# BerserkerMother/Video-Summarization

Measured on AMD Instinct MI355X. Metric: frames/sec scored (whole node), synthetic [B,T=1024,D=1024], higher is better.
Workload: dtype f32; 1 GPU; configs[2]: B=64 videos x T=1024 frames x D=1024 per GPU, scorer cfg M-A (heads 4, d_model 256, layers 4), logits + hidden state; global_batch=64, parallelism=videos sharded over 1 GPU(s), no all_gather of scores

## Files before the change

video-summarization_amd/csrc/vs_forward_plan.h:

```cpp
#pragma once
#include <stddef.h>

#include <cstdio>
#include <string>

#include "vs_scorer.h"

struct VskOptions {
    int skinny_rows;
    int lp_min_rows;
    int train_lp_min_rows;
    int lp_min_rows_fused;
    int attn_w64;
    int lp_store32;
    int lp_mlp_unfused;
    int lp_tail_unfused;
    int lp_qkv_unfused;
    int lp_tile256;
    int lp_embed_unfused;
    int exact_unfused;
    int mlp_abl;
    int attn_w64_checked;
    int attn_w64_abl;
};

enum { VSK_STORE16 = 16, VSK_A16 = 32, VSK_F16 = 64 };

enum { VSW_FRAGMENTS = 1, VSW_F16X3 = 2, VSW_BF16 = 4, VSW_ROWS16 = 8 };

inline bool vsk_mlp_bf16_supported(int d) { return d == 256; }
inline bool vsk_gemm16_supported(int M, int N, int K) { return M > 0 && N > 0 && N % 32 == 0 && K >= 32 && K % 32 == 0; }
inline bool vsk_layer_fused_supported(int M, int d, int skinny_rows) { return d == 256 && M > skinny_rows && M <= (1 << 20); }

enum VsArith { VS_ARITH_EXACT = 0, VS_ARITH_BF16 = 1, VS_ARITH_F16X3 = 2 };
enum VsEmbedForm {
    VS_EMBED_CLS,
    VS_EMBED_BF16_QKV,
    VS_EMBED_SPLITK,
    VS_EMBED_GEMM,
};
enum VsAttentionKernel {
    VS_ATT_PACKED,
    VS_ATT_DH256,
    VS_ATT_SPLITKV,
    VS_ATT_LOWPREC,
    VS_ATT_EXACT,
};
enum VsLayerForm {
    VS_LAYER_RING,
    VS_LAYER_BF16_TAIL,
    VS_LAYER_BF16_MLP,
    VS_LAYER_EXACT_PAIR,
    VS_LAYER_STAGES,
};
enum VsLnForm {
    VS_LN_NONE,
    VS_LN_SPLITK_ROWS,
    VS_LN_GEMM_ROWS,
    VS_LN_FUSED,
};

struct VsForwardIn {
    int d_model, num_heads, num_layers, in_features, max_len;
    int norm_width;
    bool has_pe, has_b_embed;
    int B, T;
    unsigned flags;
    bool cls, packed;
};

struct VsForwardPlan {
    int T, M;
    VsArith linear, attention_arith;
    unsigned families;
    VsEmbedForm embed;
    VsAttentionKernel attention;
    VsLayerForm layer;
    VsLnForm ln1, ln2;
    bool qkv16, ffn16;
    bool next_qkv;
    size_t kv_stride;
    int mode_linear;
    int mode_qkv;
    int mode_ffn;
    int mode_attention;

    bool tail_writes_qkv() const { return next_qkv || layer == VS_LAYER_EXACT_PAIR; }
};

inline int vs_attention_prec(unsigned flags) { return (flags & VS_FLAG_F16X3_ATTENTION) ? 2 : (flags & VS_FLAG_BF16_ATTENTION) ? 1 : 0; }

inline int vs_forward_plan(const VsForwardIn &in, const VskOptions &opt, VsForwardPlan *plan, std::string *err) {
    char msg[192];
    auto fail = [&](int code) { *err = msg; return code; };
    const int d = in.d_model, H = in.num_heads, dh = d / H;
    const unsigned flags = in.flags;
    if (!in.packed && in.has_pe && in.T > in.max_len) {
        snprintf(msg, sizeof msg, "T=%d exceeds the positional table (max_len=%d)", in.T, in.max_len);
        return fail(VS_ERR_INVALID);
    }
    if (in.cls && in.packed) { snprintf(msg, sizeof msg, "packed batches have no class-token form"); return fail(VS_ERR_INVALID); }
    const int T = in.T + (in.cls ? 1 : 0);
    if ((long long)in.B * T > (1ll << 30)) { snprintf(msg, sizeof msg, "B*T too large"); return fail(VS_ERR_INVALID); }
    if ((flags & VS_FLAG_BF16_LINEAR) && (flags & VS_FLAG_F16X3_LINEAR)) {
        snprintf(msg, sizeof msg, "VS_FLAG_BF16_LINEAR and VS_FLAG_F16X3_LINEAR are exclusive");
        return fail(VS_ERR_INVALID);
    }
    if ((flags & (VS_FLAG_BF16_ATTENTION | VS_FLAG_F16X3_ATTENTION)) && dh != 32 && dh != 64 && !((flags & VS_FLAG_BF16_ATTENTION) && dh == 128)) {
        snprintf(msg, sizeof msg, "VS_FLAG_BF16_ATTENTION needs head_dim 32, 64 or 128, VS_FLAG_F16X3_ATTENTION 32 or 64 (got %d)", dh);
        return fail(VS_ERR_INVALID);
    }
    if ((flags & VS_FLAG_BF16_ATTENTION) && (flags & VS_FLAG_F16X3_ATTENTION)) {
        snprintf(msg, sizeof msg, "VS_FLAG_BF16_ATTENTION and VS_FLAG_F16X3_ATTENTION are exclusive");
        return fail(VS_ERR_INVALID);
    }

    VsForwardPlan p{};
    p.T = T;
    p.M = in.B * T;
    const int M = p.M;
    const bool embedded = in.norm_width != d;
    const int aprec = vs_attention_prec(flags);
    p.attention_arith = (VsArith)aprec;
    const bool fused_ok = !embedded && vsk_mlp_bf16_supported(d) && aprec == 1 && !opt.lp_store32 && !opt.lp_mlp_unfused;
    const int lp_min_rows = fused_ok && opt.lp_min_rows_fused < opt.lp_min_rows ? opt.lp_min_rows_fused
                                                                               : opt.lp_min_rows;
    p.linear = (flags & VS_FLAG_F16X3_LINEAR) ? VS_ARITH_F16X3 : ((flags & VS_FLAG_BF16_LINEAR) && M > lp_min_rows) ? VS_ARITH_BF16 : VS_ARITH_EXACT;
    const bool bf16 = p.linear == VS_ARITH_BF16;
    const bool splitk = (flags & VS_FLAG_SPLITK) && !bf16 && !in.packed && !in.cls && M <= opt.skinny_rows && (d == 128 || d == 256 || d == 512);
    const int rows_min = in.cls ? in.B * in.T : M;
    p.families = 0;
    if (bf16) p.families = VSW_BF16;
    else if (rows_min <= opt.skinny_rows) p.families = p.linear == VS_ARITH_F16X3 ? VSW_F16X3 : VSW_FRAGMENTS;
    if (bf16 && d > 256) p.families |= VSW_ROWS16;
    p.ffn16 = bf16 && d <= 256 && !embedded && !opt.lp_store32;
    p.qkv16 = p.ffn16 && aprec == 1;
    const bool mlp16 = bf16 && !embedded && vsk_mlp_bf16_supported(d) && !opt.lp_mlp_unfused && !opt.lp_store32;
    const bool ring = bf16 && aprec == 1 && !in.packed && d > 256 && !opt.lp_store32 && vsk_gemm16_supported(M, d, d);
    p.kv_stride = (p.qkv16 || ring) ? (size_t)M * d / 2 : (size_t)M * d;
    p.next_qkv = mlp16 && p.qkv16 && !opt.lp_qkv_unfused;
    const bool exact_fused = p.linear == VS_ARITH_EXACT && aprec == 0 && !embedded && !splitk && !opt.exact_unfused &&
                             vsk_layer_fused_supported(M, d, opt.skinny_rows) && d % H == 0 && dh % 32 == 0;

    p.embed = in.cls ? VS_EMBED_CLS
            : bf16 && in.has_b_embed && p.next_qkv && in.num_layers > 0 && !opt.lp_embed_unfused ? VS_EMBED_BF16_QKV
            : splitk && in.in_features % 1024 == 0 ? VS_EMBED_SPLITK
            : VS_EMBED_GEMM;
    p.attention = in.packed ? VS_ATT_PACKED
                : dh == 256 ? VS_ATT_DH256
                : splitk && aprec != 1 && (dh == 32 || dh == 64 || dh == 128) ? VS_ATT_SPLITKV
                : aprec ? VS_ATT_LOWPREC
                : VS_ATT_EXACT;
    const VsLnForm ln = (d > 256 || embedded) ? VS_LN_GEMM_ROWS : VS_LN_FUSED;
    p.ln1 = p.ln2 = VS_LN_NONE;
    if (ring) p.layer = VS_LAYER_RING;
    else if (mlp16 && p.qkv16 && !opt.lp_tail_unfused) p.layer = VS_LAYER_BF16_TAIL;
    else if (exact_fused) p.layer = VS_LAYER_EXACT_PAIR;
    else {
        p.layer = mlp16 ? VS_LAYER_BF16_MLP : VS_LAYER_STAGES;
        p.ln1 = splitk && d >= 256 ? VS_LN_SPLITK_ROWS : ln;
        if (!mlp16) p.ln2 = splitk ? VS_LN_SPLITK_ROWS : ln;
    }
    p.mode_linear = p.linear;
    p.mode_qkv = p.qkv16 ? (1 | VSK_STORE16) : p.linear;
    p.mode_ffn = p.ffn16 ? (1 | VSK_STORE16) : p.linear;
    p.mode_attention = (p.qkv16 || ring) ? (1 | VSK_STORE16) : aprec;
    *plan = p;
    return VS_OK;
}

inline int vs_packed_waves(int dh, int aprec, long long r8, long long r4) {
    if (dh == 128) return aprec == 1 ? 8 : 4;
    return (!(aprec != 0 && dh == 32) && r8 * 100 <= r4 * 105) ? 8 : 4;
}
```

video-summarization_amd/csrc/vs_kernels.h:

```cpp
#pragma once
#include <hip/hip_runtime.h>
#include <stdint.h>

#include "vs_forward_plan.h"

int vsk_linear(const float *A, const float *W, const float *Wf, const float *bias, float *C, int M, int N, int K,
               int relu, const float *pe, int T, int bf16, hipStream_t st);
int vsk_linear_gate(const float *A, const float *W, const float *Wf, const float *bias, const float *gate, float scale,
                    float *C, int M, int N, int K, hipStream_t st, int bf16 = 0);
int vsk_linear_relu_dropout(const float *A, const float *W, const float *Wf, const float *bias, float *C, int M, int N,
                            int K, unsigned long long seed, unsigned site, float p, hipStream_t st, int bf16 = 0);
int vsk_pack_fragments(const float *W, float *Wf, int N, int K, hipStream_t st);
int vsk_pack_fragments_f16x3(const float *W, float *Wh, int N, int K, hipStream_t st);
int vsk_qkv(const float *h, const float *Wqkv, const float *Wf, const float *bqkv, float *qkv, int B, int T, int d,
            int H, int bf16, hipStream_t st, float qscale = 1.0f);
int vsk_attention(const float *q, const float *k, const float *v, const uint8_t *mask, float *out,
                  int B, int H, int T, int dh, float scale, hipStream_t st);
int vsk_attention_packed(const float *q, const float *k, const float *v, float *out, int H, int Mtot, int dh,
                         float scale, const int *cu, const int *work, int nwork, int nw, int prec, hipStream_t st);
float vsk_attention_qscale(float scale);
int vsk_attention_bf16(const float *q, const float *k, const float *v, const uint8_t *mask, float *out,
                       int B, int H, int T, int dh, float scale, int prec, hipStream_t st);
int vsk_attention_bf16_w64(const void *q, const void *k, const void *v, const uint8_t *mask, void *out, int B, int H, int T,
                           hipStream_t st);
int vsk_attention_bf16_w64_packed(const void *q, const void *k, const void *v, void *out, int H, int Mtot, const int *cu,
                                  const int *work, int nwork, hipStream_t st);
size_t vsk_attention_probs_workspace_bytes(int B, int H, int T);
int vsk_attention_probs(const float *q, const float *k, const uint8_t *mask, float *maps, float *received, float *entropy,
                        int B, int H, int T, int dh, float scale, void *workspace, hipStream_t st);
int vsk_linear_res_ln(const float *A, const float *W, const float *Wf, const float *bias, const float *res,
                      const float *gamma, const float *beta, float *out, int M, int N, int K,
                      const float *score_w, const float *score_b, int num_classes, int sigmoid,
                      float *scores, int bf16, hipStream_t st);
int vsk_outproj_ln_fc1(const float *att, const float *Wo, const float *bo, const float *res, const float *gamma, const float *beta,
                       float *h1, const float *W1, const float *b1, float *hidden, int M, int d, hipStream_t st);
int vsk_fc2_ln_qkv(const float *hidden, const float *W2, const float *b2, const float *res, const float *gamma, const float *beta,
                   float *out, const float *Wqkv, const float *bqkv, float *qkv, int B, int T, int d, int H, hipStream_t st);
int vsk_rows_res_ln(const float *a, const float *res, const float *gamma, const float *beta, float *out, int M, int d,
                    const float *score_w, const float *score_b, int num_classes, int sigmoid, float *scores,
                    hipStream_t st, void *out16 = nullptr, int dn = 0,
                    int nsplit = 0, const float *pbias = nullptr);
struct VskMatJobs {
    enum { MAX = 24 };
    const float *in[MAX];
    float *out[MAX];
    int rows[MAX], cols[MAX];
    int n;
};
int vsk_pack_fragments_batch(const VskMatJobs &jobs, hipStream_t st);
int vsk_attention_splitkv(const float *q, const float *k, const float *v, const uint8_t *mask, float *out,
                          int B, int H, int T, int dh, float scale, hipStream_t st);
int vsk_linear_parts(const float *A, const float *Wf, float *parts, int M, int N, int K, int nsplit, hipStream_t st,
                     int f16x3 = 0);
int vsk_sum_parts_pe(const float *parts, int nsplit, const float *bias, const float *pe, int T, float *out, int M, int N, hipStream_t st);
int vsk_diag_attention(const float *q, const float *k, const float *v, float *out, int B, int H, int T, float scale,
                       unsigned long long *diag, hipStream_t st);
int vsk_diag_attention_lp(const float *q, const float *k, const float *v, float *out, int B, int H, int T, float scale,
                          int prec, unsigned long long *diag, hipStream_t st);
int vsk_diag_gemm(const float *A, const float *W, const float *bias, float *C, int M, int N, int K,
                  int grid, unsigned long long *diag, hipStream_t st);
size_t vsk_mlp_bf16_image_bytes(int d);
int vsk_pack_mlp_bf16(const float *Wo, const float *W1, const float *W2, void *img, int d, hipStream_t st);
struct VskNextQkv {
    const void *img;
    const float *bqkv;
    void *qkv16;
    int T, H;
    float qscale;
};
size_t vsk_embed_bf16_image_bytes(int d, int K);
int vsk_pack_embed_bf16(const float *W, void *img, int d, int K, hipStream_t st);
int vsk_embed_bf16(const float *x, const void *img, const float *bias, const float *pe, int T, float *out, int M, int d, int K,
                   const VskNextQkv *next, hipStream_t st);
size_t vsk_qkv_bf16_image_bytes(int d);
int vsk_pack_qkv_bf16(const float *Wqkv, void *img, int d, hipStream_t st);
int vsk_mlp_bf16(const float *h, const void *att16, const float *bo, const float *gamma1, const float *beta1,
                 const void *img, const float *b1, const float *b2,
                 const float *gamma, const float *beta, float *out, int M, int d,
                 const float *score_w, const float *score_b, int num_classes, int sigmoid, float *scores,
                 const VskNextQkv *next, hipStream_t st);
int vsk_plan_packed(const int *lengths_dev, int B, int qb, int *cu, int *work, int work_cap, hipStream_t st);
int vsk_gather_rows(const float *pe, const int *cu, int B, int tmax, int d, float *rows, hipStream_t st);
enum { VSK_COPY_MAX_SEGS = 20 };
struct VskCopySegs {
    const float *src[VSK_COPY_MAX_SEGS];
    float *dst[VSK_COPY_MAX_SEGS];
    unsigned n[VSK_COPY_MAX_SEGS];
    int count;
};
int vsk_copy_segments(const VskCopySegs &segs, hipStream_t st);
// ... 11 lines not shown
```

video-summarization_amd/csrc/vs_kernels.hip:

```cpp
#include "vs_train_device.h"
#include "vs_kernels.h"
#include "vs_launch.h"

namespace {

enum { EPI_BIAS = 0, EPI_RELU = 1, EPI_PE = 2, EPI_QKV = 3,
       EPI_GATE = 4,
       EPI_RELU_DROP = 5 };
struct EpiArgs {
    unsigned long long seed;
    unsigned site;
    float p;
    float scale;
};

__device__ __forceinline__ unsigned long long stamp() { return vs_stamp(); }

template <int EPI, int NWM = 2, int DIAG = 0, int NJ = 2, int PREC = 0, int C16 = 0, int KW = 32, int A16 = 0>
__global__ __launch_bounds__(128 * NWM, 2) void gemm_nt_128(
    const float *__restrict__ A, const float *__restrict__ W, const float *__restrict__ bias,
    float *__restrict__ C, int M, int N, int K, const float *__restrict__ pe, int T, int H, int dh,
    unsigned long long *__restrict__ diag = nullptr, EpiArgs ea = EpiArgs{0ull, 0u, 0.f, 0.f}) {
    static_assert(KW == 32 || (KW == 64 && (PREC == 1 || PREC == 3)), "64-wide k-tiles exist for the 16-bit operands only");
    static_assert(A16 == 0 || PREC == 1 || PREC == 3, "16-bit-stored A belongs to the 16-bit operand modes");
// ... 499 lines not shown
        part[t] = half_sum(s);
    }
    if (r == 0) {
#pragma unroll
        for (int t = 0; t < 16; ++t) red[wc * 64 + 32 * wr + acc_row(t, h)] = part[t];
    }
    __syncthreads();
#pragma unroll
    for (int t = 0; t < 16; ++t) {
        const int rl = 32 * wr + acc_row(t, h);
        const float rstd = 1.0f / sqrtf((red[rl] + red[64 + rl]) * (1.0f / N) + 1e-5f);
        const int row = m0 + rl;
#pragma unroll
        for (int j = 0; j < NB; ++j) {
            const float y = acc[j][t] * rstd * gj[j] + bej[j];
            acc[j][t] = y;
            if (row < M) out[(size_t)row * N + cbase + 32 * j] = y;
        }
    }
    if (score_w != nullptr) {
        for (int c = 0; c < num_classes; ++c) {
            __syncthreads();
            float wj[NB];
#pragma unroll
            for (int j = 0; j < NB; ++j) wj[j] = score_w[(size_t)c * N + cbase + 32 * j];
#pragma unroll
            for (int t = 0; t < 16; ++t) {
                float s = 0.f;
#pragma unroll
                for (int j = 0; j < NB; ++j) s += acc[j][t] * wj[j];
                part[t] = half_sum(s);
            }
            if (r == 0) {
#pragma unroll
                for (int t = 0; t < 16; ++t) red[wc * 64 + 32 * wr + acc_row(t, h)] = part[t];
            }
            __syncthreads();
            if (tid < 64) {
                const int row = m0 + tid;
                if (row < M) {
                    float s = red[tid] + red[64 + tid] + score_b[c];
                    if (sigmoid) s = 1.0f / (1.0f + expf(-s));
                    scores[(size_t)row * num_classes + c] = s;
                }
            }
        }
    }
}

struct LnTail {
    const float *W2, *b2;
    float *C2;
    int T, H, dhs;
};

template <int NT, int PREC, int A16, int DIAG, int TAIL>
__device__ __forceinline__ void ln_rows_tiles(
    const float *__restrict__ A, const float *__restrict__ W, const float *__restrict__ bias,
    const float *__restrict__ res, const float *__restrict__ gamma, const float *__restrict__ beta,
    float *__restrict__ out, int M, int K,
    const float *__restrict__ score_w, const float *__restrict__ score_b, int num_classes,
    int sigmoid, float *__restrict__ scores, unsigned long long *__restrict__ diag, const LnTail tl) {
    static_assert(TAIL == 0 || (NT == 8 && PREC == 0 && DIAG == 0), "the register-fed tail exists for exact fp32 at d_model 256");
    constexpr int BM = 128, N = 32 * NT, BK = 16, LD = BK + 4;
    constexpr int WL = (N * BK / 4 + 255) / 256;
    constexpr int TN2 = TAIL == 2 ? 3 * N : 4 * N;
    __shared__ __attribute__((aligned(16))) float smem[2 * (BM + N) * LD + 4 * N + (TAIL != 0 ? TN2 : 0)];
    float *gam_s = smem + 2 * (BM + N) * LD, *bet_s = gam_s + N, *sw_s = bet_s + N, *bias_s = sw_s + N;
    float *bias2_s = bias_s + N;

    const int tid = threadIdx.x, lane = tid & 63, wave = tid >> 6;
    const int r = lane & 31, h = lane >> 5;
    const int ntiles = (M + BM - 1) / BM;
    const int nk = K / BK;

    constexpr float SC = PREC == 2 ? F16X3_WS : 1.0f;
    for (int i = tid; i < N; i += 256) { gam_s[i] = gamma[i]; bet_s[i] = beta[i]; bias_s[i] = bias[i] * SC; }
    if constexpr (TAIL != 0)
        for (int i = tid; i < TN2; i += 256) bias2_s[i] = tl.b2[i];

    const int lrow = tid >> 2, lc4 = (tid & 3) * 4;
    f32x4 pa[2], pw[WL];
    u32x2 pa16[2];
    const float *aptr[2], *wptr[WL];
    const unsigned short *aptr16[2];
#pragma unroll
    for (int i = 0; i < WL; ++i) {
        int wrow = lrow + 64 * i; wrow = wrow < N ? wrow : N - 1;
        wptr[i] = W + (size_t)wrow * K + lc4;
    }
    static_assert(PREC != 0 || N % 64 == 0, "the exact-fp32 staging map covers W without a guard");
    __amdgpu_buffer_rsrc_t ars = __builtin_amdgcn_make_buffer_rsrc(const_cast<float *>(A), 0, 0, 0x00020000);
    const __amdgpu_buffer_rsrc_t wrs = __builtin_amdgcn_make_buffer_rsrc(const_cast<float *>(W), 0, N * K * 4, 0x00020000);
    int aoff[2], woff[WL];
#pragma unroll
    for (int i = 0; i < WL; ++i) woff[i] = ((lrow + 64 * i) * K + lc4) * 4;
    auto gload = [&](int i, int kb) __attribute__((always_inline)) {
        if (i < 2) pa[i] = __builtin_bit_cast(f32x4, __builtin_amdgcn_raw_buffer_load_b128(ars, aoff[i], kb, 0));
        else pw[i - 2] = __builtin_bit_cast(f32x4, __builtin_amdgcn_raw_buffer_load_b128(wrs, woff[i - 2], kb, 0));
    };
    constexpr int LDB = 12;
    auto stage = [&](int buf) __attribute__((always_inline)) {
        float *As = smem + buf * (BM + N) * LD, *Ws = As + BM * LD;
        if constexpr (PREC == 2) {
#pragma unroll
            for (int i = 0; i < 2; ++i) {
                u32x2 hi, lo;
                split_f16x4((const float *)&pa[i], hi, lo);
                *(u32x2 *)&As[(lrow + 64 * i) * LD + lc4 / 2] = hi;
                *(u32x2 *)&As[(lrow + 64 * i) * LD + 8 + lc4 / 2] = lo;
            }
#pragma unroll
            for (int i = 0; i < WL; ++i)
                if (lrow + 64 * i < N) {
                    u32x2 hi, lo;
                    const f32x4 ws = pw[i] * F16X3_WS;
                    split_f16x4((const float *)&ws, hi, lo);
                    *(u32x2 *)&Ws[(lrow + 64 * i) * LD + lc4 / 2] = hi;
                    *(u32x2 *)&Ws[(lrow + 64 * i) * LD + 8 + lc4 / 2] = lo;
                }
        } else if constexpr (PREC == 1) {
#pragma unroll
            for (int i = 0; i < 2; ++i) {
                u32x2 u;
                if constexpr (A16 != 0) u = pa16[i];
                else { u[0] = pack_bf16(pa[i][0], pa[i][1]); u[1] = pack_bf16(pa[i][2], pa[i][3]); }
                *(u32x2 *)&As[(lrow + 64 * i) * LDB + lc4 / 2] = u;
            }
#pragma unroll
            for (int i = 0; i < WL; ++i)
// ... 39 lines not shown
        const float *wp = smem + TWB + (kt & 1) * TBUF + r * 36 + 4 * h;
        float *wd = smem + TWB + ((kt + 1) & 1) * TBUF + r2 * 36 + c2;
        f32x4 fw[3];
        fw[0] = *(const f32x4 *)wp;
        fw[1] = *(const f32x4 *)(wp + 32 * 36);
        __builtin_amdgcn_sched_barrier(0);
#pragma unroll
        for (int t = 0; t < 16; ++t) {
            const int g = t / 4, jj = t % 4;
            if (t + 2 < 16) fw[(t + 2) % 3] = *(const f32x4 *)(wp + 32 * ((t + 2) % 4) * 36 + 8 * ((t + 2) / 4));
            if (t < 4) tail_load(t, nsoff);
            if (t >= 12) *(f32x4 *)(wd + 32 * (t - 12) * 36) = pw2[t - 12];
#pragma unroll
            for (int s2 = 0; s2 < 4; ++s2) U[jj] = MFMA32(fw[t % 3][s2], acc[kt][4 * g + s2], U[jj]);
            __builtin_amdgcn_sched_group_barrier(0x008, 1, 0);
            if (t + 2 < 16) __builtin_amdgcn_sched_group_barrier(0x100, 1, 0);
            if (t < 4) __builtin_amdgcn_sched_group_barrier(0x020, 1, 0);
            __builtin_amdgcn_sched_group_barrier(0x008, 3, 0);
            if (t >= 12) __builtin_amdgcn_sched_group_barrier(0x200, 1, 0);
            __builtin_amdgcn_sched_barrier(0);
        }
        __syncthreads();
    };

    unsigned long long dsum[3] = {0, 0, 0}, tbegin = 0, tq = 0, ktiles = 0;
    if constexpr (DIAG != 0) tbegin = stamp();
    for (int tile = blockIdx.x; tile < ntiles; tile += gridDim.x) {
        if constexpr (DIAG != 0) tq = stamp();
        const int m0 = tile * BM;
        int row = m0 + 32 * wave + r;
        const bool row_ok = row < M;
        row = row_ok ? row : M - 1;
#pragma unroll
        for (int i = 0; i < 2; ++i) {
            int ar = m0 + lrow + 64 * i; ar = ar < M ? ar : M - 1;
            if constexpr (A16 != 0) {
                aptr16[i] = (const unsigned short *)A + (size_t)ar * K + lc4;
                pa16[i] = *(const u32x2 *)aptr16[i];
            } else if constexpr (PREC == 0) {
                aoff[i] = ((ar - m0) * K + lc4) * 4;
            } else {
                aptr[i] = A + (size_t)ar * K + lc4;
                pa[i] = *(const f32x4 *)aptr[i];
            }
        }
        if constexpr (PREC == 0) {
            ars = __builtin_amdgcn_make_buffer_rsrc(const_cast<float *>(A + (size_t)m0 * K), 0, (M - m0 < BM ? M - m0 : BM) * K * 4, 0x00020000);
#pragma unroll
            for (int i = 0; i < 2 + WL; ++i) gload(i, 0);
        } else {
#pragma unroll
            for (int i = 0; i < WL; ++i) pw[i] = *(const f32x4 *)wptr[i];
        }
        {
            const float *rp = res + (size_t)row * N + 4 * h;
#pragma unroll
            for (int j = 0; j < NT; ++j)
#pragma unroll
                for (int q = 0; q < 4; ++q) {
                    f32x4 rv = *(const f32x4 *)(rp + 32 * j + 8 * q);
                    if constexpr (PREC == 2) rv *= SC;
#pragma unroll
                    for (int e = 0; e < 4; ++e) acc[j][4 * q + e] = rv[e];
                }
        }
        __syncthreads();
        stage(0);
        __syncthreads();
        if constexpr (DIAG != 0) { dsum[2] += stamp() - tq; ktiles += nk; }

        for (int kt = 0; kt < nk; ++kt) {
            const int kn = kt + 1 < nk ? kt + 1 : kt;
            const float *As = smem + (kt & 1) * (BM + N) * LD, *Ws = As + BM * LD;
            if constexpr (PREC == 2) {
                const float *arow = As + (32 * wave + r) * LD + 4 * h;
                const f16x8 ah = __builtin_bit_cast(f16x8, *(const u32x4 *)arow);
                const f16x8 al = __builtin_bit_cast(f16x8, *(const u32x4 *)(arow + 8));
#pragma unroll
                for (int i = 0; i < 2; ++i) pa[i] = *(const f32x4 *)(aptr[i] + kn * BK);
#pragma unroll
                for (int i = 0; i < WL; ++i) pw[i] = *(const f32x4 *)(wptr[i] + kn * BK);
#pragma unroll
                for (int j = 0; j < NT; ++j) {
                    const float *wrow = Ws + (32 * j + r) * LD + 4 * h;
                    const f16x8 wh = __builtin_bit_cast(f16x8, *(const u32x4 *)wrow);
                    const f16x8 wl = __builtin_bit_cast(f16x8, *(const u32x4 *)(wrow + 8));
                    acc[j] = MFMA_F16(wl, ah, acc[j]);
                    acc[j] = MFMA_F16(wh, al, acc[j]);
                    acc[j] = MFMA_F16(wh, ah, acc[j]);
                }
                stage((kt + 1) & 1);
                __syncthreads();
                continue;
            }
            if constexpr (PREC == 1) {
                const bf16x8 fa = __builtin_bit_cast(bf16x8, *(const u32x4 *)(As + (32 * wave + r) * LDB + 4 * h));
#pragma unroll
                for (int i = 0; i < 2; ++i) {
                    if constexpr (A16 != 0) pa16[i] = *(const u32x2 *)(aptr16[i] + kn * BK);
                    else pa[i] = *(const f32x4 *)(aptr[i] + kn * BK);
                }
#pragma unroll
                for (int i = 0; i < WL; ++i) pw[i] = *(const f32x4 *)(wptr[i] + kn * BK);
#pragma unroll
                for (int j = 0; j < NT; ++j) {
                    const bf16x8 fw = __builtin_bit_cast(bf16x8, *(const u32x4 *)(Ws + (32 * j + r) * LDB + 4 * h));
                    acc[j] = MFMA_BF16(fw, fa, acc[j]);
                }
                stage((kt + 1) & 1);
                __syncthreads();
                continue;
            }
            const float *ap = As + (32 * wave + r) * LD + 4 * h;
            const float *wp = Ws + r * LD + 4 * h;
            constexpr int NS = 2 * NT, NL = 2 + WL;
            constexpr int LPS = (NL + NT - 1) / NT;
            constexpr int WB = NS - (NL + LPS - 1) / LPS;
            static_assert(BK == 16 && (NL + LPS - 1) / LPS <= NT, "loads and LDS writes of a k-tile occupy distinct steps");
            f32x4 fa[2], fw[3];
            fa[0] = *(const f32x4 *)ap;
            fw[0] = *(const f32x4 *)wp;
            fw[1] = *(const f32x4 *)(wp + 32 * LD);
            fa[1] = *(const f32x4 *)(ap + 8);
            __builtin_amdgcn_sched_barrier(0);
#pragma unroll
            for (int t = 0; t < NS; ++t) {
                const int g = t / NT, j = t % NT;
                if (t + 2 < NS) fw[(t + 2) % 3] = *(const f32x4 *)(wp + 32 * ((t + 2) % NT) * LD + 8 * ((t + 2) / NT));
                int nld = 0, nwr = 0;
#pragma unroll
                for (int q = 0; q < LPS; ++q) {
                    const int il = t * LPS + q, iw = (t - WB) * LPS + q;
                    if (il < NL) { gload(il, kn * (BK * 4)); ++nld; }
                    if (t >= WB && iw < NL) {
                        float *Ad = smem + ((kt + 1) & 1) * (BM + N) * LD, *Wd = Ad + BM * LD;
                        if (iw < 2) *(f32x4 *)&Ad[(lrow + 64 * iw) * LD + lc4] = pa[iw];
                        else *(f32x4 *)&Wd[(lrow + 64 * (iw - 2)) * LD + lc4] = pw[iw - 2];
                        ++nwr;
                    }
                }
#pragma unroll
                for (int s2 = 0; s2 < 4; ++s2) acc[j] = MFMA32(fw[t % 3][s2], fa[g][s2], acc[j]);
                __builtin_amdgcn_sched_group_barrier(0x008, 1, 0);
                if (t + 2 < NS) __builtin_amdgcn_sched_group_barrier(0x100, 1, 0);
#pragma unroll
                for (int q = 0; q < LPS; ++q)
                    if (q < nld) __builtin_amdgcn_sched_group_barrier(0x020, 1, 0);
                __builtin_amdgcn_sched_group_barrier(0x008, 3, 0);
#pragma unroll
                for (int q = 0; q < LPS; ++q)
                    if (q < nwr) __builtin_amdgcn_sched_group_barrier(0x200, 1, 0);
                __builtin_amdgcn_sched_barrier(0);
            }
            if constexpr (DIAG != 0) {
                const unsigned long long tb = stamp();
                __syncthreads();
                dsum[0] += stamp() - tb;
            } else
                __syncthreads();
        }
        if constexpr (DIAG != 0) tq = stamp();
        if constexpr (TAIL != 0) {
#pragma unroll
            for (int i = 0; i < 4; ++i) tail_load(i, tail_soff(0, 0));
        }

        float sum = 0.f;
#pragma unroll
        for (int j = 0; j < NT; ++j) {
            float pj = 0.f;
#pragma unroll
            for (int q = 0; q < 4; ++q) {
                const f32x4 bv = *(const f32x4 *)&bias_s[32 * j + 8 * q + 4 * h];
#pragma unroll
                for (int e = 0; e < 4; ++e) { acc[j][4 * q + e] += bv[e]; pj += acc[j][4 * q + e]; }
            }
            sum += pj;
        }
        sum = pair_sum(sum);
        const float mean = sum * (1.0f / N);
        float sq = 0.f;
#pragma unroll
        for (int j = 0; j < NT; ++j) {
            float pj = 0.f;
#pragma unroll
            for (int t = 0; t < 16; ++t) { const float c = acc[j][t] - mean; acc[j][t] = c; pj += c * c; }
            sq += pj;
        }
        sq = pair_sum(sq);
        const float rstd = 1.0f / sqrtf(sq * (1.0f / N) + 1e-5f * (SC * SC));
        float *tp = smem + wave * (32 * 36);
        const int trow = lane >> 3, tc4 = (lane & 7) * 4;
#pragma unroll
        for (int j = 0; j < NT; ++j) {
#pragma unroll
            for (int q = 0; q < 4; ++q) {
                const f32x4 gv = *(const f32x4 *)&gam_s[32 * j + 8 * q + 4 * h];
                const f32x4 bv = *(const f32x4 *)&bet_s[32 * j + 8 * q + 4 * h];
                f32x4 y;
#pragma unroll
                for (int e = 0; e < 4; ++e) { y[e] = acc[j][4 * q + e] * rstd * gv[e] + bv[e]; acc[j][4 * q + e] = y[e]; }
                *(f32x4 *)&tp[r * 36 + 8 * q + 4 * h] = y;
            }
#pragma unroll
            for (int pq = 0; pq < 4; ++pq) {
                const f32x4 v = *(const f32x4 *)&tp[(trow + 8 * pq) * 36 + tc4];
                const int orow = m0 + 32 * wave + trow + 8 * pq;
                if (orow < M) *(f32x4 *)(out + (size_t)orow * N + 32 * j + tc4) = v;
            }
        }
        if (score_w != nullptr) {
            for (int c = 0; c < num_classes; ++c) {
                __syncthreads();
                for (int i = tid; i < N; i += 256) sw_s[i] = score_w[(size_t)c * N + i];
                __syncthreads();
                float dot = 0.f;
#pragma unroll
                for (int j = 0; j < NT; ++j) {
                    float pj = 0.f;
#pragma unroll
                    for (int q = 0; q < 4; ++q) {
                        const f32x4 wv = *(const f32x4 *)&sw_s[32 * j + 8 * q + 4 * h];
#pragma unroll
                        for (int e = 0; e < 4; ++e) pj += acc[j][4 * q + e] * wv[e];
                    }
                    dot += pj;
                }
                dot = pair_sum(dot);
                if (h == 0 && row_ok) {
                    float sc = dot + score_b[c];
                    if (sigmoid) sc = 1.0f / (1.0f + expf(-sc));
                    scores[(size_t)row * num_classes + c] = sc;
                }
            }
        }
        if constexpr (DIAG != 0) dsum[1] += stamp() - tq;
        if constexpr (TAIL != 0) {
            tail_stage(0);
            int rowoff[4];
            __amdgpu_buffer_rsrc_t crs;
            if constexpr (TAIL == 1) {
                crs = __builtin_amdgcn_make_buffer_rsrc(tl.C2 + (size_t)m0 * TN2, 0, (M - m0 < BM ? M - m0 : BM) * TN2 * 4, 0x00020000);
#pragma unroll
                for (int p = 0; p < 4; ++p) rowoff[p] = ((32 * wave + trow + 8 * p) * TN2 + tc4) * 4;
            } else {
                crs = __builtin_amdgcn_make_buffer_rsrc(tl.C2, 0, 0, 0x00020000);
#pragma unroll
                for (int p = 0; p < 4; ++p) {
                    const int orow = m0 + 32 * wave + trow + 8 * p;
                    const int bb = orow / tl.T, tt = orow - bb * tl.T;
                    rowoff[p] = orow < M ? (((bb * tl.H * tl.T + tt) << tl.dhs) + tc4) * 4 : (int)0x80000000;
                }
            }
            bias_mfma(0);
            __syncthreads();
            for (int c = 0; c < TNC; ++c) {
                const int cn = c + 1 < TNC ? c + 1 : c;
                static_for<8>([&](auto ktc) __attribute__((always_inline)) {
                    constexpr int kt = decltype(ktc)::value;
                    tail_step(ktc, kt < 7 ? tail_soff(c, kt + 1) : tail_soff(cn, 0));
                });
                if constexpr (TAIL == 2) {
                    const int which = c >> 1;
                    crs = __builtin_amdgcn_make_buffer_rsrc(tl.C2 + (size_t)which * M * N, 0, M * N * 4, 0x00020000);
                }
#pragma unroll
                for (int jj = 0; jj < 4; ++jj) {
                    __builtin_amdgcn_sched_barrier(0);
#pragma unroll
                    for (int q = 0; q < 4; ++q) {
                        f32x4 v;
#pragma unroll
                        for (int e = 0; e < 4; ++e) v[e] = TAIL == 1 ? relu1(U[jj][4 * q + e]) : U[jj][4 * q + e];
                        *(f32x4 *)&tp[r * 36 + 8 * q + 4 * h] = v;
                    }
                    int soff;
                    if constexpr (TAIL == 1) soff = (TCH * c + 32 * jj) * 4;
                    else {
                        const int cc = (TCH * c + 32 * jj) & (N - 1), head = cc >> tl.dhs, e0 = cc - (head << tl.dhs);
                        soff = (((head * tl.T) << tl.dhs) + e0) * 4;
                    }
#pragma unroll
                    for (int p = 0; p < 4; ++p) {
                        const f32x4 v = *(const f32x4 *)&tp[(trow + 8 * p) * 36 + tc4];
                        __builtin_amdgcn_raw_buffer_store_b128(__builtin_bit_cast(u32x4, v), crs, rowoff[p], soff, 0);
                    }
                }
                __builtin_amdgcn_sched_barrier(0);
                bias_mfma(cn);
            }
        }
    }
    if constexpr (DIAG != 0) {
        if (diag != nullptr && lane == 0) {
            unsigned long long *o = diag + ((size_t)blockIdx.x * 4 + wave) * 8;
            o[0] = dsum[0]; o[1] = dsum[1]; o[2] = dsum[2]; o[3] = 0; o[4] = 0;
            o[5] = stamp() - tbegin; o[6] = ktiles; o[7] = tbegin;
        }
    }
}

template <int NT, int PREC = 0, int A16 = 0, int DIAG = 0>
__global__ __launch_bounds__(256, 2) void gemm_ln_rows(
    const float *__restrict__ A, const float *__restrict__ W, const float *__restrict__ bias,
    const float *__restrict__ res, const float *__restrict__ gamma, const float *__restrict__ beta,
    float *__restrict__ out, int M, int K,
    const float *__restrict__ score_w, const float *__restrict__ score_b, int num_classes,
    int sigmoid, float *__restrict__ scores, unsigned long long *__restrict__ diag = nullptr) {
    ln_rows_tiles<NT, PREC, A16, DIAG, 0>(A, W, bias, res, gamma, beta, out, M, K, score_w, score_b, num_classes, sigmoid, scores, diag,
                                          LnTail{nullptr, nullptr, nullptr, 0, 0, 0});
}

__global__ __launch_bounds__(256, 2) void layer_outproj_ln_fc1(
    const float *__restrict__ A, const float *__restrict__ W, const float *__restrict__ bias,
    const float *__restrict__ res, const float *__restrict__ gamma, const float *__restrict__ beta,
    float *__restrict__ out, int M, int K, const float *__restrict__ W1, const float *__restrict__ b1, float *__restrict__ hidden) {
    ln_rows_tiles<8, 0, 0, 0, 1>(A, W, bias, res, gamma, beta, out, M, K, nullptr, nullptr, 0, 0, nullptr, nullptr,
                                 LnTail{W1, b1, hidden, 0, 0, 0});
}
__global__ __launch_bounds__(256, 2) void layer_fc2_ln_qkv(
    const float *__restrict__ A, const float *__restrict__ W, const float *__restrict__ bias,
    const float *__restrict__ res, const float *__restrict__ gamma, const float *__restrict__ beta,
    float *__restrict__ out, int M, int K, const float *__restrict__ Wqkv, const float *__restrict__ bqkv, float *__restrict__ qkv,
    int T, int H, int dhs) {
    ln_rows_tiles<8, 0, 0, 0, 2>(A, W, bias, res, gamma, beta, out, M, K, nullptr, nullptr, 0, 0, nullptr, nullptr,
                                 LnTail{Wqkv, bqkv, qkv, T, H, dhs});
}

__device__ __forceinline__ void skinny_mainloop(f32x16 &acc, const float *__restrict__ ap,
                                                const float *__restrict__ wp, int K) {
    f32x4 a[4][4], w[4][4];
    auto load = [&](int set, int off) __attribute__((always_inline)) {
#pragma unroll
        for (int g = 0; g < 4; ++g) {
            a[set][g] = *(const f32x4 *)(ap + off + 8 * g);
            w[set][g] = *(const f32x4 *)(wp + off + 8 * g);
        }
    };
    auto mma = [&](int set) __attribute__((always_inline)) {
#pragma unroll
        for (int g = 0; g < 4; ++g)
#pragma unroll
            for (int st = 0; st < 4; ++st) acc = MFMA32(w[set][g][st], a[set][g][st], acc);
    };
    const int nc = K / 32;
    load(0, 0); load(1, 32); load(2, 64);
    for (int c = 0; c < nc - 4; c += 4) {
        load(3, 96);  mma(0);
        load(0, 128); mma(1);
        load(1, 160); mma(2);
        load(2, 192); mma(3);
        ap += 128; wp += 128;
    }
    load(3, 96);
    mma(0); mma(1); mma(2); mma(3);
}

template <int EPI>
__global__ __launch_bounds__(256) void skinny_gemm(
    const float *__restrict__ A, const float *__restrict__ W, const float *__restrict__ bias,
    float *__restrict__ C, int M, int N, int K, const float *__restrict__ pe, int T, int H, int dh, EpiArgs ea) {
    const int lane = threadIdx.x & 63, wave = threadIdx.x >> 6, r = lane & 31, h = lane >> 5;
    const int m0 = blockIdx.x * 32, n0 = blockIdx.y * 128 + 32 * wave;
    if (n0 >= N) return;
    const int row = m0 + r;
    const int arow = row < M ? row : M - 1;
    const float *ap = A + (size_t)arow * K + 4 * h, *wp = W + (size_t)(n0 + r) * K + 4 * h;
    const f32x16 zero = {0.f, 0.f, 0.f, 0.f, 0.f, 0.f, 0.f, 0.f, 0.f, 0.f, 0.f, 0.f, 0.f, 0.f, 0.f, 0.f};
    f32x16 acc = MFMA32(h == 0 ? bias[n0 + r] : 0.f, 1.0f, zero);
    skinny_mainloop(acc, ap, wp, K);
    if (row >= M) return;
// ... 953 lines not shown
        return 0;
    }
    if (N <= 256 && N % 32 == 0) {
        int blocks = persistent_blocks((M + 127) / 128);
        if (blocks < 0) return (int)hipErrorInvalidDevice;
        if (blocks > (M + 127) / 128) blocks = (M + 127) / 128;
        if (!vsk_pick_int<2, 4, 6, 8>(N / 32, [&](auto NT) {
                hipLaunchKernelGGL((gemm_ln_rows<NT(), 0>), dim3(blocks), dim3(256), 0, st, A, W, bias, res, gamma, beta, out, M, K,
                                   score_w, score_b, num_classes, sigmoid, scores);
            }))
            return -1;
        VSK_CHECK_LAUNCH();
        return 0;
    }
    const int blocks = (M + 63) / 64;
    if (!vsk_pick_int<1, 2, 3, 4, 5, 6, 7, 8>(N / 64, [&](auto NB) {
            if (bf16 == 2)
                hipLaunchKernelGGL((gemm_res_ln<NB(), 2>), dim3(blocks), dim3(256), 0, st, A, W, bias, res, gamma, beta, out, M, K,
                                   score_w, score_b, num_classes, sigmoid, scores);
            else
                hipLaunchKernelGGL((gemm_res_ln<NB(), 0>), dim3(blocks), dim3(256), 0, st, A, W, bias, res, gamma, beta, out, M, K,
                                   score_w, score_b, num_classes, sigmoid, scores);
        }))
        return -1;
    VSK_CHECK_LAUNCH();
    return 0;
}


int vsk_outproj_ln_fc1(const float *att, const float *Wo, const float *bo, const float *res, const float *gamma, const float *beta,
                       float *h1, const float *W1, const float *b1, float *hidden, int M, int d, hipStream_t st) {
    if (!vsk_layer_fused_supported(M, d, skinny_max_rows())) return -1;
    int blocks = persistent_blocks((M + 127) / 128);
    if (blocks < 0) return (int)hipErrorInvalidDevice;
    if (blocks > (M + 127) / 128) blocks = (M + 127) / 128;
    hipLaunchKernelGGL(layer_outproj_ln_fc1, dim3(blocks), dim3(256), 0, st, att, Wo, bo, res, gamma, beta, h1, M, d, W1, b1, hidden);
    VSK_CHECK_LAUNCH();
    return 0;
}

int vsk_fc2_ln_qkv(const float *hidden, const float *W2, const float *b2, const float *res, const float *gamma, const float *beta,
                   float *out, const float *Wqkv, const float *bqkv, float *qkv, int B, int T, int d, int H, hipStream_t st) {
    const int M = B * T;
    if (!vsk_layer_fused_supported(M, d, skinny_max_rows()) || H <= 0 || d % H || (d / H) % 32) return -1;
    int dhs = 5;
    while ((1 << dhs) < d / H) ++dhs;
    int blocks = persistent_blocks((M + 127) / 128);
    if (blocks < 0) return (int)hipErrorInvalidDevice;
    if (blocks > (M + 127) / 128) blocks = (M + 127) / 128;
    hipLaunchKernelGGL(layer_fc2_ln_qkv, dim3(blocks), dim3(256), 0, st, hidden, W2, b2, res, gamma, beta, out, M, 4 * d, Wqkv, bqkv, qkv, T, H, dhs);
    VSK_CHECK_LAUNCH();
    return 0;
}
```

video-summarization_amd/csrc/vs_scorer.cpp:

```cpp
#include "vs_scorer.h"
#include "vs_inspect.h"

#include <hip/hip_runtime.h>

#include <atomic>
#include <cmath>
#include <cstdarg>
#include <cstdio>
#include <cstdlib>
#include <cstring>
#include <mutex>
#include <string>
#include <vector>

#include "vs_kernels.h"
#include "vs_train_kernels.h"
#include "vs_weights_impl.h"

namespace {

thread_local std::string g_err;

int fail(int code, const char *fmt, ...) {
    char buf[512];
// ... 342 lines not shown

namespace {
struct PackedInfo {
    const float *pe_rows;
    const int *cu;
    const int *work;
    int nwork, nw;
};

struct InspectHook {
    const int32_t *layers;
    int n_layers;
    float *maps, *received, *entropy;
    void *workspace;
};

int forward_core(const vs_weights *w, const float *x, const uint8_t *key_pad_mask, int32_t B,
                 int32_t T, uint32_t flags, float *scores, float *hidden, void *workspace,
                 size_t workspace_bytes, void *stream, const PackedInfo *pk, const float *cls = nullptr,
                 const InspectHook *ins = nullptr) {
    if (!w || !x || !scores) return fail(VS_ERR_INVALID, "weights/x/scores is NULL");
    if (B <= 0 || T <= 0) return fail(VS_ERR_INVALID, "B=%d T=%d", B, T);
    const vs_model_desc &D = w->desc;
    const int Tf = T;
    const int sig = (flags & VS_FLAG_SIGMOID) ? 1 : 0;
    const VsForwardIn in{D.d_model, D.num_heads, D.num_layers, D.in_features, D.max_len, w->dn(), w->has_pe, w->has_b_embed,
                         B, Tf, flags, cls != nullptr, pk != nullptr};
    VsForwardPlan plan;
    if (int rc = vs_forward_plan(in, vsk_options(), &plan, &g_err)) return rc;
    T = plan.T;
    const size_t need_core = vs_scorer_workspace_bytes(w, B, T);
    const size_t need = need_core + (cls ? align_up((size_t)B * T, 256) : 0);
    if (!workspace || workspace_bytes < need)
        return fail(VS_ERR_WORKSPACE, "workspace %zu bytes < %zu needed", workspace_bytes, need);
    if (((uintptr_t)workspace & 255) || ((uintptr_t)x & 15) || (hidden && ((uintptr_t)hidden & 15)) || (cls && ((uintptr_t)cls & 15)))
        return fail(VS_ERR_INVALID, "workspace must be 256-byte, x/hidden/cls_token 16-byte aligned");
    vsw_order(w, stream);
    if (plan.families) if (int rc = vsw_ensure(w, plan.families, stream)) return rc;

    hipStream_t st = (hipStream_t)stream;
    const int d = D.d_model, H = D.num_heads, L = D.num_layers, M = plan.M;
    const size_t md = align_up((size_t)M * d * sizeof(float), 256) / sizeof(float);
    float *ws = (float *)workspace;
    float *h0 = ws, *h1 = ws + md, *qkv = ws + 2 * md, *att = ws + 5 * md, *ffn = ws + 6 * md;
    void *h16 = ffn + 2 * md;
    const size_t kv = plan.kv_stride;
    const int dn = w->dn();
    const float scale = 1.0f / sqrtf((float)dn);
    const float qs = vsk_attention_qscale(scale);
    const bool f16x3 = plan.linear == VS_ARITH_F16X3;
    auto frag = [&](size_t f, size_t h) { return w->p(f16x3 ? h : f); };
    const float *pe_rows = pk ? pk->pe_rows : (w->has_pe ? w->p(w->pe) : nullptr);
    {
        StageScope ps(VS_STAGE_EMBED, st);
        switch (plan.embed) {
        case VS_EMBED_CLS: {
            VS_LAUNCH(vsk_linear(x, w->p(w->embed_w), frag(w->f_embed_w, w->h_embed_w), w->p(w->embed_b), h1, B * Tf, d,
                                 D.in_features, 0, pe_rows, Tf, plan.mode_linear, st));
            uint8_t *mask1 = key_pad_mask ? (uint8_t *)workspace + need_core : nullptr;
            VS_LAUNCH(vsk_insert_cls(h1, cls, key_pad_mask, h0, mask1, B, Tf, d, st));
            key_pad_mask = mask1;
        } break;
        case VS_EMBED_BF16_QKV: {
            const LayerOff &N = w->layers[0];
            const VskNextQkv nq{w->p(N.b_qkv), w->p(N.bqkv), qkv, T, H, qs};
            VS_LAUNCH(vsk_embed_bf16(x, w->p(w->b_embed), w->p(w->embed_b), pe_rows, T, h0, M, d, D.in_features, &nq, st));
        } break;
        case VS_EMBED_SPLITK:
            VS_LAUNCH(vsk_linear_parts(x, frag(w->f_embed_w, w->h_embed_w), qkv, M, d, D.in_features, 8, st, f16x3));
            VS_LAUNCH(vsk_sum_parts_pe(qkv, 8, w->p(w->embed_b), pe_rows, T, h0, M, d, st));
            break;
        case VS_EMBED_GEMM:
            VS_LAUNCH(vsk_linear(x, w->p(w->embed_w), frag(w->f_embed_w, w->h_embed_w), w->p(w->embed_b), h0, M, d, D.in_features, 0,
                                 pe_rows, T, plan.mode_linear, st));
            break;
        }
    }
    if (plan.layer == VS_LAYER_RING) VS_LAUNCH(vsk_to_bf16(h0, h16, (size_t)M * d, st));
    for (int l = 0; l < L; ++l) {
        const LayerOff &P = w->layers[l];
        const bool last = l == L - 1;
        float *dst = (last && hidden) ? hidden : h0;
        const float *head_w = last ? w->p(w->final_w) : nullptr, *head_b = last ? w->p(w->final_b) : nullptr;
        float *head_out = last ? scores : nullptr;
        VskNextQkv nq{}, *next = nullptr;
        if (plan.next_qkv && !last) {
            const LayerOff &N = w->layers[l + 1];
            nq = VskNextQkv{w->p(N.b_qkv), w->p(N.bqkv), qkv, T, H, qs};
            next = &nq;
        }
        if (plan.layer == VS_LAYER_RING) {
            StageScope ps(VS_STAGE_QKV, st);
            VS_LAUNCH(vsk_gemm16(h16, w->p(P.r_wqkv), w->p(P.bqkv), qkv, M, 3 * d, d, 3, 1, T, H, d / H, qs, st));
        } else if (l == 0 ? plan.embed != VS_EMBED_BF16_QKV : !plan.tail_writes_qkv()) {
            StageScope ps(VS_STAGE_QKV, st);
            VS_LAUNCH(vsk_qkv(h0, w->p(P.wqkv), frag(P.f_wqkv, P.h_wqkv), w->p(P.bqkv), qkv, B, T, d, H, plan.mode_qkv, st,
                              plan.qkv16 ? qs : 1.0f));
        }
        if (ins) {
            for (int i = 0; i < ins->n_layers; ++i) {
                if (ins->layers[i] != l) continue;
                const size_t rows = (size_t)B * H * T;
                VS_LAUNCH(vsk_attention_probs(qkv, qkv + kv, key_pad_mask, ins->maps ? ins->maps + i * rows * T : nullptr,
                                              ins->received ? ins->received + i * rows : nullptr,
                                              ins->entropy ? ins->entropy + i * rows : nullptr, B, H, T, d / H, scale, ins->workspace, st));
            }
        }
        {
            StageScope ps(VS_STAGE_ATTENTION, st);
            switch (plan.attention) {
            case VS_ATT_PACKED:
                VS_LAUNCH(vsk_attention_packed(qkv, qkv + kv, qkv + 2 * kv, att, H, M, d / H, scale, pk->cu, pk->work, pk->nwork, pk->nw,
                                               plan.mode_attention, st));
                break;
            case VS_ATT_DH256:
                VS_LAUNCH(vst_attention_fwd(qkv, qkv + kv, qkv + 2 * kv, key_pad_mask, att, ffn, B, H, T, 256, scale, 0ull, 0u, 0.f, st, nullptr));
                break;
            case VS_ATT_SPLITKV:
                VS_LAUNCH(vsk_attention_splitkv(qkv, qkv + kv, qkv + 2 * kv, key_pad_mask, att, B, H, T, d / H, scale, st));
                break;
            case VS_ATT_LOWPREC:
                VS_LAUNCH(vsk_attention_bf16(qkv, qkv + kv, qkv + 2 * kv, key_pad_mask, att, B, H, T, d / H, scale, plan.mode_attention, st));
                break;
            case VS_ATT_EXACT:
                VS_LAUNCH(vsk_attention(qkv, qkv + kv, qkv + 2 * kv, key_pad_mask, att, B, H, T, d / H, scale, st));
                break;
            }
        }
        if (plan.ln1 != VS_LN_NONE) {
            StageScope ps(VS_STAGE_OUTPROJ_LN, st);
            switch (plan.ln1) {
            case VS_LN_SPLITK_ROWS:
                VS_LAUNCH(vsk_linear_parts(att, frag(P.f_wo, P.h_wo), qkv, M, d, d, 2, st, f16x3));
                VS_LAUNCH(vsk_rows_res_ln(qkv, h0, w->p(P.ln1g), w->p(P.ln1b), h1, M, d, nullptr, nullptr, 0, 0, nullptr, st, nullptr, dn,
                                          2, w->p(P.bo)));
                break;
            case VS_LN_GEMM_ROWS:
                VS_LAUNCH(vsk_linear(att, w->p(P.wo), frag(P.f_wo, P.h_wo), w->p(P.bo), qkv, M, d, d, 0, nullptr, 1, plan.mode_linear, st));
                VS_LAUNCH(vsk_rows_res_ln(qkv, h0, w->p(P.ln1g), w->p(P.ln1b), h1, M, d, nullptr, nullptr, 0, 0, nullptr, st, nullptr, dn));
                break;
            default:
                VS_LAUNCH(vsk_linear_res_ln(att, w->p(P.wo), frag(P.f_wo, P.h_wo), w->p(P.bo), h0, w->p(P.ln1g), w->p(P.ln1b), h1, M, d, d,
                                            nullptr, nullptr, 0, 0, nullptr, plan.mode_qkv, st));
            }
        }
        switch (plan.layer) {
        case VS_LAYER_RING: {
// ... 444 lines not shown
```

Before: 12.08 million frames/s.

## Fuse exact fp32 embedding GEMM with positional add and layer-0 QKV projection

Adds a TAIL==3 variant of the row-tile kernel that computes the embedding linear (bias seeded via MFMA), adds positional encodings, stores h0, then runs the register-fed QKV tail for layer 0 in the same persistent kernel. The plan enables it for the exact fp32 fused-layer path, so the separate layer-0 QKV launch and the reread of h0 are dropped. In exchange the kernel gets more complex, with a larger K loop over in_features, and it skips the LayerNorm code in this tail mode.

```diff
diff --git a/video-summarization_amd/csrc/vs_forward_plan.h b/video-summarization_amd/csrc/vs_forward_plan.h
--- a/video-summarization_amd/csrc/vs_forward_plan.h
+++ b/video-summarization_amd/csrc/vs_forward_plan.h
@@ -31,6 +31,7 @@
 inline bool vsk_mlp_bf16_supported(int d) { return d == 256; }
 inline bool vsk_gemm16_supported(int M, int N, int K) { return M > 0 && N > 0 && N % 32 == 0 && K >= 32 && K % 32 == 0; }
 inline bool vsk_layer_fused_supported(int M, int d, int skinny_rows) { return d == 256 && M > skinny_rows && M <= (1 << 20); }
+inline bool vsk_embed_qkv_supported(int in_features) { return in_features >= 16 && in_features % 16 == 0 && in_features <= (1 << 20); }
 
 enum VsArith { VS_ARITH_EXACT = 0, VS_ARITH_BF16 = 1, VS_ARITH_F16X3 = 2 };
 enum VsEmbedForm {
@@ -84,8 +85,11 @@
     int mode_qkv;
     int mode_ffn;
     int mode_attention;
+    bool embed_exact_qkv = false;
 
     bool tail_writes_qkv() const { return next_qkv || layer == VS_LAYER_EXACT_PAIR; }
+    bool embed_writes_qkv() const { return embed == VS_EMBED_BF16_QKV || embed_exact_qkv; }
+    bool qkv_written_before(int l) const { return l == 0 ? embed_writes_qkv() : tail_writes_qkv(); }
 };
 
 inline int vs_attention_prec(unsigned flags) { return (flags & VS_FLAG_F16X3_ATTENTION) ? 2 : (flags & VS_FLAG_BF16_ATTENTION) ? 1 : 0; }
@@ -146,6 +150,7 @@
             : bf16 && in.has_b_embed && p.next_qkv && in.num_layers > 0 && !opt.lp_embed_unfused ? VS_EMBED_BF16_QKV
             : splitk && in.in_features % 1024 == 0 ? VS_EMBED_SPLITK
             : VS_EMBED_GEMM;
+    p.embed_exact_qkv = p.embed == VS_EMBED_GEMM && exact_fused && in.num_layers > 0 && vsk_embed_qkv_supported(in.in_features);
     p.attention = in.packed ? VS_ATT_PACKED
                 : dh == 256 ? VS_ATT_DH256
                 : splitk && aprec != 1 && (dh == 32 || dh == 64 || dh == 128) ? VS_ATT_SPLITKV
diff --git a/video-summarization_amd/csrc/vs_kernels.h b/video-summarization_amd/csrc/vs_kernels.h
--- a/video-summarization_amd/csrc/vs_kernels.h
+++ b/video-summarization_amd/csrc/vs_kernels.h
@@ -36,6 +36,8 @@
                        float *h1, const float *W1, const float *b1, float *hidden, int M, int d, hipStream_t st);
 int vsk_fc2_ln_qkv(const float *hidden, const float *W2, const float *b2, const float *res, const float *gamma, const float *beta,
                    float *out, const float *Wqkv, const float *bqkv, float *qkv, int B, int T, int d, int H, hipStream_t st);
+int vsk_embed_pe_qkv(const float *x, const float *We, const float *be, const float *pe, float *h0, const float *Wqkv, const float *bqkv,
+                     float *qkv, int B, int T, int d, int in_features, int H, hipStream_t st);
 int vsk_rows_res_ln(const float *a, const float *res, const float *gamma, const float *beta, float *out, int M, int d,
                     const float *score_w, const float *score_b, int num_classes, int sigmoid, float *scores,
                     hipStream_t st, void *out16 = nullptr, int dn = 0,
diff --git a/video-summarization_amd/csrc/vs_kernels.hip b/video-summarization_amd/csrc/vs_kernels.hip
--- a/video-summarization_amd/csrc/vs_kernels.hip
+++ b/video-summarization_amd/csrc/vs_kernels.hip
@@ -575,6 +575,7 @@
     const float *W2, *b2;
     float *C2;
     int T, H, dhs;
+    const float *pe;
 };
 
 template <int NT, int PREC, int A16, int DIAG, int TAIL>
@@ -587,7 +588,7 @@
     static_assert(TAIL == 0 || (NT == 8 && PREC == 0 && DIAG == 0), "the register-fed tail exists for exact fp32 at d_model 256");
     constexpr int BM = 128, N = 32 * NT, BK = 16, LD = BK + 4;
     constexpr int WL = (N * BK / 4 + 255) / 256;
-    constexpr int TN2 = TAIL == 2 ? 3 * N : 4 * N;
+    constexpr int TN2 = TAIL >= 2 ? 3 * N : 4 * N;
     __shared__ __attribute__((aligned(16))) float smem[2 * (BM + N) * LD + 4 * N + (TAIL != 0 ? TN2 : 0)];
     float *gam_s = smem + 2 * (BM + N) * LD, *bet_s = gam_s + N, *sw_s = bet_s + N, *bias_s = sw_s + N;
     float *bias2_s = bias_s + N;
@@ -598,7 +599,10 @@
     const int nk = K / BK;
 
     constexpr float SC = PREC == 2 ? F16X3_WS : 1.0f;
-    for (int i = tid; i < N; i += 256) { gam_s[i] = gamma[i]; bet_s[i] = beta[i]; bias_s[i] = bias[i] * SC; }
+    if constexpr (TAIL == 3) {
+        for (int i = tid; i < N; i += 256) bias_s[i] = bias[i];
+    } else
+        for (int i = tid; i < N; i += 256) { gam_s[i] = gamma[i]; bet_s[i] = beta[i]; bias_s[i] = bias[i] * SC; }
     if constexpr (TAIL != 0)
         for (int i = tid; i < TN2; i += 256) bias2_s[i] = tl.b2[i];
 
@@ -744,7 +748,7 @@
 #pragma unroll
             for (int i = 0; i < WL; ++i) pw[i] = *(const f32x4 *)wptr[i];
         }
-        {
+        if constexpr (TAIL != 3) {
             const float *rp = res + (size_t)row * N + 4 * h;
 #pragma unroll
             for (int j = 0; j < NT; ++j)
@@ -759,6 +763,14 @@
         __syncthreads();
         stage(0);
         __syncthreads();
+        if constexpr (TAIL == 3) {
+            const f32x16 zero = {0.f, 0.f, 0.f, 0.f, 0.f, 0.f, 0.f, 0.f, 0.f, 0.f, 0.f, 0.f, 0.f, 0.f, 0.f, 0.f};
+#pragma unroll
+            for (int j = 0; j < NT; ++j) {
+                const float bv = bias_s[32 * j + r];
+                acc[j] = MFMA32(h == 0 ? bv : 0.f, 1.0f, zero);
+            }
+        }
         if constexpr (DIAG != 0) { dsum[2] += stamp() - tq; ktiles += nk; }
 
         for (int kt = 0; kt < nk; ++kt) {
@@ -857,6 +869,39 @@
             for (int i = 0; i < 4; ++i) tail_load(i, tail_soff(0, 0));
         }
 
+        float *tp = smem + wave * (32 * 36);
+        const int trow = lane >> 3, tc4 = (lane & 7) * 4;
+        if constexpr (TAIL == 3) {
+            if (tl.pe != nullptr) {
+                const float *pp = tl.pe + (size_t)(row % tl.T) * N + 4 * h;
+#pragma unroll
+                for (int j = 0; j < NT; ++j)
+#pragma unroll
+                    for (int q = 0; q < 4; ++q) {
+                        const f32x4 pv = *(const f32x4 *)(pp + 32 * j + 8 * q);
+#pragma unroll
+                        for (int e = 0; e < 4; ++e) acc[j][4 * q + e] += pv[e];
+                    }
+            }
+#pragma unroll
+            for (int j = 0; j < NT; ++j) {
+                __builtin_amdgcn_sched_barrier(0);
+#pragma unroll
+                for (int q = 0; q < 4; ++q) {
+                    f32x4 y;
+#pragma unroll
+                    for (int e = 0; e < 4; ++e) y[e] = acc[j][4 * q + e];
+                    *(f32x4 *)&tp[r * 36 + 8 * q + 4 * h] = y;
+                }
+#pragma unroll
+                for (int pq = 0; pq < 4; ++pq) {
+                    const f32x4 v = *(const f32x4 *)&tp[(trow + 8 * pq) * 36 + tc4];
+                    const int orow = m0 + 32 * wave + trow + 8 * pq;
+                    if (orow < M) *(f32x4 *)(out + (size_t)orow * N + 32 * j + tc4) = v;
+                }
+            }
+            __builtin_amdgcn_sched_barrier(0);
+        } else {
         float sum = 0.f;
 #pragma unroll
         for (int j = 0; j < NT; ++j) {
@@ -881,8 +926,6 @@
         }
         sq = pair_sum(sq);
         const float rstd = 1.0f / sqrtf(sq * (1.0f / N) + 1e-5f * (SC * SC));
-        float *tp = smem + wave * (32 * 36);
-        const int trow = lane >> 3, tc4 = (lane & 7) * 4;
 #pragma unroll
         for (int j = 0; j < NT; ++j) {
 #pragma unroll
@@ -925,6 +968,7 @@
                     scores[(size_t)row * num_classes + c] = sc;
                 }
             }
+        }
         }
         if constexpr (DIAG != 0) dsum[1] += stamp() - tq;
         if constexpr (TAIL != 0) {
@@ -952,7 +996,7 @@
                     constexpr int kt = decltype(ktc)::value;
                     tail_step(ktc, kt < 7 ? tail_soff(c, kt + 1) : tail_soff(cn, 0));
                 });
-                if constexpr (TAIL == 2) {
+                if constexpr (TAIL >= 2) {
                     const int which = c >> 1;
                     crs = __builtin_amdgcn_make_buffer_rsrc(tl.C2 + (size_t)which * M * N, 0, M * N * 4, 0x00020000);
                 }
@@ -1009,6 +1053,13 @@
     float *__restrict__ out, int M, int K, const float *__restrict__ W1, const float *__restrict__ b1, float *__restrict__ hidden) {
     ln_rows_tiles<8, 0, 0, 0, 1>(A, W, bias, res, gamma, beta, out, M, K, nullptr, nullptr, 0, 0, nullptr, nullptr,
                                  LnTail{W1, b1, hidden, 0, 0, 0});
+}
+__global__ __launch_bounds__(256, 2) void embed_pe_qkv(
+    const float *__restrict__ x, const float *__restrict__ We, const float *__restrict__ be, const float *__restrict__ pe,
+    float *__restrict__ h0, int M, int K, const float *__restrict__ Wqkv, const float *__restrict__ bqkv, float *__restrict__ qkv,
+    int T, int H, int dhs) {
+    ln_rows_tiles<8, 0, 0, 0, 3>(x, We, be, nullptr, nullptr, nullptr, h0, M, K, nullptr, nullptr, 0, 0, nullptr, nullptr,
+                                 LnTail{Wqkv, bqkv, qkv, T, H, dhs, pe});
 }
 __global__ __launch_bounds__(256, 2) void layer_fc2_ln_qkv(
     const float *__restrict__ A, const float *__restrict__ W, const float *__restrict__ bias,
@@ -2068,3 +2119,18 @@
     VSK_CHECK_LAUNCH();
     return 0;
 }
+
+int vsk_embed_pe_qkv(const float *x, const float *We, const float *be, const float *pe, float *h0, const float *Wqkv, const float *bqkv,
+                     float *qkv, int B, int T, int d, int in_features, int H, hipStream_t st) {
+    const int M = B * T;
+    if (!vsk_layer_fused_supported(M, d, skinny_max_rows()) || !vsk_embed_qkv_supported(in_features) || H <= 0 || d % H || (d / H) % 32)
+        return -1;
+    int dhs = 5;
+    while ((1 << dhs) < d / H) ++dhs;
+    int blocks = persistent_blocks((M + 127) / 128);
+    if (blocks < 0) return (int)hipErrorInvalidDevice;
+    if (blocks > (M + 127) / 128) blocks = (M + 127) / 128;
+    hipLaunchKernelGGL(embed_pe_qkv, dim3(blocks), dim3(256), 0, st, x, We, be, pe, h0, M, in_features, Wqkv, bqkv, qkv, T, H, dhs);
+    VSK_CHECK_LAUNCH();
+    return 0;
+}
diff --git a/video-summarization_amd/csrc/vs_scorer.cpp b/video-summarization_amd/csrc/vs_scorer.cpp
--- a/video-summarization_amd/csrc/vs_scorer.cpp
+++ b/video-summarization_amd/csrc/vs_scorer.cpp
@@ -418,7 +418,7 @@
     auto frag = [&](size_t f, size_t h) { return w->p(f16x3 ? h : f); };
     const float *pe_rows = pk ? pk->pe_rows : (w->has_pe ? w->p(w->pe) : nullptr);
     {
-        StageScope ps(VS_STAGE_EMBED, st);
+        StageScope ps(plan.embed_exact_qkv ? VS_STAGE_QKV : VS_STAGE_EMBED, st);
         switch (plan.embed) {
         case VS_EMBED_CLS: {
             VS_LAUNCH(vsk_linear(x, w->p(w->embed_w), frag(w->f_embed_w, w->h_embed_w), w->p(w->embed_b), h1, B * Tf, d,
@@ -437,6 +437,11 @@
             VS_LAUNCH(vsk_sum_parts_pe(qkv, 8, w->p(w->embed_b), pe_rows, T, h0, M, d, st));
             break;
         case VS_EMBED_GEMM:
+            if (plan.embed_exact_qkv) {
+                const LayerOff &N = w->layers[0];
+                VS_LAUNCH(vsk_embed_pe_qkv(x, w->p(w->embed_w), w->p(w->embed_b), pe_rows, h0, w->p(N.wqkv), w->p(N.bqkv), qkv, B, T, d,
+                                           D.in_features, H, st));
+            } else
             VS_LAUNCH(vsk_linear(x, w->p(w->embed_w), frag(w->f_embed_w, w->h_embed_w), w->p(w->embed_b), h0, M, d, D.in_features, 0,
                                  pe_rows, T, plan.mode_linear, st));
             break;
@@ -458,7 +463,7 @@
         if (plan.layer == VS_LAYER_RING) {
             StageScope ps(VS_STAGE_QKV, st);
             VS_LAUNCH(vsk_gemm16(h16, w->p(P.r_wqkv), w->p(P.bqkv), qkv, M, 3 * d, d, 3, 1, T, H, d / H, qs, st));
-        } else if (l == 0 ? plan.embed != VS_EMBED_BF16_QKV : !plan.tail_writes_qkv()) {
+        } else if (!plan.qkv_written_before(l)) {
             StageScope ps(VS_STAGE_QKV, st);
             VS_LAUNCH(vsk_qkv(h0, w->p(P.wqkv), frag(P.f_wqkv, P.h_wqkv), w->p(P.bqkv), qkv, B, T, d, H, plan.mode_qkv, st,
                               plan.qkv16 ? qs : 1.0f));
```

New measurement: 12.13 million frames/s, median of 6. No clear change (+0.5%).
